# doing-science-to-stuff/ndt

Measured on AMD Instinct MI355X. Metric: Mray/s (primary+shadow+reflect) at 1920x1080, higher is better.
Workload: dtype f64

## Files before the change

ndt_amd/csrc/ndt_api.hip:

```cpp
#include "ndt_ctx.hpp"
#include <ctype.h>


static thread_local char g_err[512] = "";
int ndt_impl::fail(int code, const char *fmt, ...)
{
    va_list ap;
    va_start(ap, fmt);
    vsnprintf(g_err, sizeof(g_err), fmt, ap);
    va_end(ap);
    return code;
}

extern "C" const char *ndt_hip_last_error(void) { return g_err; }
extern "C" int ndt_hip_abi_version(void) { return NDT_HIP_ABI_VERSION; }

extern "C" int32_t ndt_hip_shard_rows(int32_t height, int32_t row_begin, int32_t row_step)
{
    if (row_step < 1 || row_begin < 0 || row_begin >= height) return 0;
    return (height - row_begin + row_step - 1) / row_step;
}

static const NdtKernelTable *table_for(int dims)
{
    switch (dims) {
    case 3: return ndt_kernel_table_3();
    case 4: return ndt_kernel_table_4();
    case 5: return ndt_kernel_table_5();
    case 6: return ndt_kernel_table_6();
    case 7: return ndt_kernel_table_7();
    case 8: return ndt_kernel_table_8();
    case 9: return ndt_kernel_table_9();
    case 10: return ndt_kernel_table_10();
    case 11: return ndt_kernel_table_11();
    case 12: return ndt_kernel_table_12();
    default: return nullptr;
    }
}

extern "C" int ndt_hip_create(int device, ndt_hip_ctx **out)
{
    if (!out) return fail(NDT_E_INVALID, "ndt_hip_create: out is NULL");
    *out = nullptr;
    int count = 0;
    hipError_t e = hipGetDeviceCount(&count);
    if (e != hipSuccess || count <= 0)
        return fail(NDT_E_DEVICE, "no HIP device available (%s); libndt_hip has no CPU path",
                    e == hipSuccess ? "device count is 0" : hipGetErrorString(e));
    if (device < 0 || device >= count) return fail(NDT_E_INVALID, "device %d out of range (have %d)", device, count);
    HIP_TRY(hipSetDevice(device));
    hipDeviceProp_t prop;
    HIP_TRY(hipGetDeviceProperties(&prop, device));
    if (strncmp(prop.gcnArchName, "gfx950", 6) != 0)
        return fail(NDT_E_DEVICE, "device %d is %s; this library carries gfx950 code objects only", device, prop.gcnArchName);
    ndt_hip_ctx *ctx = new ndt_hip_ctx();
    ctx->device = device;
    {
        static const char *const names[] = { "hybrid_level", "stream_below", "stream_below_list", "hull_box", "face_box", "face_tree", "face_groups", "item_sets", "gate_prepass", "gate_prepass_below", "item_boxes", "leaf_history", "leaf_scan", "leaf_scan_group", "multi_path", "sample_seed", "stream_fused", "fuse_primaries", "shade_pair", "light_overlap", "light_window", "debug_levels",
                                             "exit_probe", "shade_probe", "stream_probe", "test_small_pool" };
        const char *pl = getenv("NDT_HIP_PIPELINE");
        if (pl) (void)ndt_hip_set_option(ctx, "pipeline", !strcmp(pl, "levels") ? 1 : !strcmp(pl, "stream") ? 2 : !strcmp(pl, "hybrid") ? 3 : 0);
        for (const char *nm : names) {
            char env[64] = "NDT_HIP_";
            size_t k = strlen(env);
            for (const char *q = nm; *q && k + 1 < sizeof(env); ++q) env[k++] = (char)toupper((unsigned char)*q);
            env[k] = 0;
            const char *v = getenv(env);
            if (v && *v) (void)ndt_hip_set_option(ctx, nm, !strcmp(nm, "shade_probe") ? atoll(v) + 1 : atoll(v));
        }
        if (getenv("NDT_HIP_NO_HULL_BOX")) ctx->hull_box = false;
        if (getenv("NDT_HIP_NO_FACE_BOX")) ctx->face_box = false;
        if (getenv("NDT_HIP_NO_SHADE_PAIR") && atoi(getenv("NDT_HIP_NO_SHADE_PAIR"))) ctx->shade_pair = false;
    }
    e = hipStreamCreateWithFlags(&ctx->stream, hipStreamNonBlocking);
    if (e == hipSuccess) {
        int least = 0, greatest = 0;
        e = hipDeviceGetStreamPriorityRange(&least, &greatest);
        if (e == hipSuccess) e = hipStreamCreateWithPriority(&ctx->light_stream, hipStreamNonBlocking, least);
        if (e != hipSuccess) (void)hipStreamDestroy(ctx->stream);
    }
    if (e != hipSuccess) {
        delete ctx;
        return fail(NDT_E_DEVICE, "hipStreamCreate: %s", hipGetErrorString(e));
    }
    e = hipHostMalloc((void **)&ctx->h_counters, 128 * sizeof(int), hipHostMallocDefault);
    if (e == hipSuccess) e = hipHostMalloc((void **)&ctx->h_levels, (NDT_MAX_LEVELS + 1) * sizeof(LevelRange), hipHostMallocDefault);
    if (e == hipSuccess) e = hipHostMalloc((void **)&ctx->h_mail, (NDT_MAX_LEVELS + 2) * sizeof(LevelRange), hipHostMallocMapped | hipHostMallocCoherent);
    if (e == hipSuccess) e = hipHostMalloc((void **)&ctx->h_mail_tag, (NDT_MAX_LEVELS + 2) * sizeof(unsigned long long), hipHostMallocMapped | hipHostMallocCoherent);
    if (e == hipSuccess) e = hipHostGetDevicePointer((void **)&ctx->d_mail, ctx->h_mail, 0);
    if (e == hipSuccess) e = hipHostGetDevicePointer((void **)&ctx->d_mail_tag, ctx->h_mail_tag, 0);
    if (e == hipSuccess) memset(ctx->h_mail_tag, 0, (NDT_MAX_LEVELS + 2) * sizeof(unsigned long long));
    if (e == hipSuccess) e = hipHostMalloc((void **)&ctx->h_done, 16 * sizeof(unsigned long long), hipHostMallocMapped | hipHostMallocCoherent);
    if (e == hipSuccess) e = hipHostGetDevicePointer((void **)&ctx->d_done, ctx->h_done, 0);
    if (e == hipSuccess) memset(ctx->h_done, 0, 16 * sizeof(unsigned long long));
    if (e != hipSuccess) {
        (void)hipStreamDestroy(ctx->light_stream);
        (void)hipStreamDestroy(ctx->stream);
        delete ctx;
        return fail(NDT_E_DEVICE, "hipHostMalloc: %s", hipGetErrorString(e));
    }
    *out = ctx;
    return NDT_OK;
}

extern "C" int ndt_hip_destroy(ndt_hip_ctx *ctx)
{
    if (!ctx) return NDT_OK;
    worker_stop(ctx);
    (void)hipSetDevice(ctx->device);
    (void)sync_streams(ctx);
    free_workspace(ctx);
    free_stage(ctx);
    free_async(ctx);
    if (ctx->d_shard) (void)hipFree(ctx->d_shard);
    if (ctx->d_image) (void)hipFree(ctx->d_image);
    for (auto &slot : ctx->pool)
        if (slot.first) (void)hipFree(slot.first);
    for (auto &slot : ctx->pool2)
        if (slot.first) (void)hipFree(slot.first);
    if (ctx->d_blob) (void)hipFree(ctx->d_blob);
    if (ctx->d_out) (void)hipFree(ctx->d_out);
    if (ctx->d_fit) (void)hipFree(ctx->d_fit);
    free_kd(ctx);
    free_png(ctx);
    free_jpeg(ctx);
    free_depth(ctx);
    free_ssaa(ctx);
    if (ctx->d_eyes) (void)hipFree(ctx->d_eyes);
    if (ctx->h_counters) (void)hipHostFree(ctx->h_counters);
    if (ctx->h_levels) (void)hipHostFree(ctx->h_levels);
    if (ctx->h_mail) (void)hipHostFree(ctx->h_mail);
    if (ctx->h_mail_tag) (void)hipHostFree(ctx->h_mail_tag);
    if (ctx->h_done) (void)hipHostFree(ctx->h_done);
    for (hipEvent_t ev : ctx->ev_pool) (void)hipEventDestroy(ev);
    (void)hipStreamDestroy(ctx->light_stream);
    (void)hipStreamDestroy(ctx->stream);
    delete ctx;
    return NDT_OK;
}

extern "C" int ndt_hip_set_option(ndt_hip_ctx *ctx, const char *name, int64_t value)
{
    if (!ctx || !name) return fail(NDT_E_INVALID, "NULL argument");
    const bool on = value != 0;
    if (!strcmp(name, "pipeline")) {
        if (value < 0 || value > 3) return fail(NDT_E_INVALID, "pipeline %lld", (long long)value);
        ctx->pipeline = (int)value;
    } else if (!strcmp(name, "hybrid_level")) ctx->hybrid_level = (int)value;
    else if (!strcmp(name, "stream_below")) ctx->stream_below = value;
    else if (!strcmp(name, "stream_below_list")) ctx->stream_below_list = value;
    else if (!strcmp(name, "hull_box")) ctx->hull_box = on;
    else if (!strcmp(name, "face_box")) ctx->face_box = on;
    else if (!strcmp(name, "face_tree")) ctx->face_tree = on;
    else if (!strcmp(name, "face_groups")) ctx->face_groups = on;
    else if (!strcmp(name, "item_sets")) ctx->item_sets = on;
    else if (!strcmp(name, "item_boxes")) ctx->item_boxes = on;
    else if (!strcmp(name, "gate_prepass_below")) ctx->gate_prepass_below = value;
    else if (!strcmp(name, "gate_prepass")) ctx->gate_prepass = value < 0 ? 0 : value > 2 ? 2 : (int)value;
    else if (!strcmp(name, "sample_seed")) ctx->sample_seed = value;
    else if (!strcmp(name, "leaf_scan")) ctx->leaf_scan = on;
    else if (!strcmp(name, "leaf_scan_group")) ctx->leaf_scan_group = value < 1 ? 1 : value > 64 ? 64 : (int)value;
    else if (!strcmp(name, "leaf_history")) ctx->leaf_history = value < 0 ? 0 : value > 4 ? 4 : (int)value;
    else if (!strcmp(name, "multi_path")) {
        if (value < 0 || value > 2) return fail(NDT_E_INVALID, "multi_path %lld", (long long)value);
        ctx->multi_path = (int)value;
    } else if (!strcmp(name, "stream_fused")) ctx->stream_fused = on;
    else if (!strcmp(name, "fuse_primaries")) ctx->fuse_primaries = value < 0 ? -1 : on ? 1 : 0;
    else if (!strcmp(name, "shade_pair")) ctx->shade_pair = on;
    else if (!strcmp(name, "light_overlap")) ctx->light_overlap = on;
    else if (!strcmp(name, "light_window")) {
        if (value < 0 || value > 64) return fail(NDT_E_INVALID, "light_window %lld (0 auto, 1 .. 64)", (long long)value);
        ctx->light_window = (int)value;
        if (ctx->have_scene) light_windows(ctx);
    }
    else if (!strcmp(name, "debug_levels")) ctx->debug_levels = on;
    else if (!strcmp(name, "exit_probe")) ctx->exit_probe = on;
    else if (!strcmp(name, "shade_probe")) ctx->shade_probe = (int)value - 1;
    else if (!strcmp(name, "stream_probe")) ctx->stream_probe = on;
    else if (!strcmp(name, "test_small_pool")) ctx->test_small_pool = on;
    else return fail(NDT_E_INVALID, "unknown option '%s'", name);
    return NDT_OK;
}

extern "C" void *ndt_hip_stream(ndt_hip_ctx *ctx) { return ctx ? (void *)ctx->stream : nullptr; }
extern "C" int ndt_hip_synchronize(ndt_hip_ctx *ctx)
{
    if (!ctx) return fail(NDT_E_INVALID, "ctx is NULL");
    HIP_TRY(hipSetDevice(ctx->device));
    HIP_TRY(hipStreamSynchronize(ctx->stream));
    return NDT_OK;
}

extern "C" int ndt_hip_upload_scene(ndt_hip_ctx *ctx, const ndt_flat_scene *fs)
{
    if (!ctx || !fs) return fail(NDT_E_INVALID, "NULL argument");
    if (fs->abi_version != NDT_HIP_ABI_VERSION) return fail(NDT_E_INVALID, "scene ABI %d, library ABI %d", fs->abi_version, NDT_HIP_ABI_VERSION);
    if (fs->dims < NDT_MIN_DIMS || fs->dims > NDT_MAX_DIMS)
        return fail(NDT_E_UNSUPPORTED, "%d dimensions: kernels are built for %d..%d", fs->dims, NDT_MIN_DIMS, NDT_MAX_DIMS);
    if (fs->cam_type < 0 || fs->cam_type > 2) return fail(NDT_E_UNSUPPORTED, "camera type %d", fs->cam_type);
    if (fs->cam_type != 0 && (fs->cam_local_x_off < 0 || fs->cam_local_y_off < 0 || fs->cam_local_z_off < 0))
        return fail(NDT_E_INVALID, "VR / panorama cameras need the local axes (camera.h:69-71) in the flat scene");
    if (fs->n_lights < 0 || fs->n_lights > NDT_MAX_LIGHTS) return fail(NDT_E_UNSUPPORTED, "%d lights (max %d)", fs->n_lights, NDT_MAX_LIGHTS);
    if (fs->n_objects < 0 || fs->n_items < 0 || fs->n_items > fs->n_objects) return fail(NDT_E_INVALID, "object counts");
    if (fs->n_kd_nodes < 0 || fs->n_inf < 0 || fs->n_leaf_refs < 0) return fail(NDT_E_INVALID, "kd-tree counts");
    if (fs->n_objects > 0 && !fs->objects) return fail(NDT_E_INVALID, "objects is NULL");
    if (fs->n_lights > 0 && !fs->lights) return fail(NDT_E_INVALID, "lights is NULL");
    if (!fs->vecs) return fail(NDT_E_INVALID, "vecs is NULL");
    HIP_TRY(hipSetDevice(ctx->device));
    ctx->have_scene = false;
    int rc = build_blob(ctx, fs);
    if (rc) return rc;
    ctx->dims = fs->dims;
    ctx->kt = table_for(fs->dims);
    if (!ctx->kt) return fail(NDT_E_UNSUPPORTED, "no kernels for %d dimensions", fs->dims);
    HIP_TRY(sync_streams(ctx));
    if (ctx->d_blob_words < ctx->blob.size()) {
        if (ctx->d_blob) HIP_TRY(hipFree(ctx->d_blob));
        ctx->d_blob = nullptr;
        HIP_TRY(hipMalloc((void **)&ctx->d_blob, ctx->blob.size() * sizeof(double)));
        ctx->d_blob_words = ctx->blob.size();
    }
    HIP_TRY(hipMemcpyAsync(ctx->d_blob, ctx->blob.data(), ctx->blob.size() * sizeof(double), hipMemcpyHostToDevice, ctx->stream));
    HIP_TRY(hipStreamSynchronize(ctx->stream));
    ctx->aperture_radius = fs->cam_aperture_radius;
    ctx->have_scene = true;
    if (ctx->debug_levels)
        fprintf(stderr, "ndt_hip: scene blob: %d-D, %d items / %d objects, %d kd nodes of depth %d; %d words staged by the trace kernels (%d KB), %d in all; tier %d, %d mask word(s)\n",
                ctx->dims, ctx->sd.n_items, ctx->sd.n_objects, ctx->sd.n_kd_nodes, ctx->sd.kd_depth, ctx->sd.trace_words, ctx->sd.trace_words / 128,
                ctx->sd.total_words, ctx->tier, ctx->sd.mask_words);
    return NDT_OK;
}

__global__ void k_quantize(const double *rgba, unsigned char *out, long long n_values)
{
    const long long i = (long long)blockIdx.x * blockDim.x + threadIdx.x;
    if (i >= n_values) return;
    const double d = rgba[i];
    double m = (1.0 < d) ? 1.0 : d;
    m = (0.0 > m) ? 0.0 : m;
    out[i] = (unsigned char)(sqrt(m) * 255);
}

extern "C" int ndt_hip_quantize_device(ndt_hip_ctx *ctx, const void *d_rgba, void *d_rgba8, int64_t n_pixels)
{
    if (!ctx || !d_rgba || !d_rgba8 || n_pixels < 0) return fail(NDT_E_INVALID, "bad argument");
    HIP_TRY(hipSetDevice(ctx->device));
    const long long n = n_pixels * 4;
    if (n == 0) return NDT_OK;
    hipLaunchKernelGGL(k_quantize, dim3((unsigned)((n + 255) / 256)), dim3(256), 0, ctx->stream, (const double *)d_rgba,
                       (unsigned char *)d_rgba8, n);
    HIP_TRY(hipGetLastError());
    return NDT_OK;
// ... 77 lines not shown
```

ndt_amd/csrc/ndt_ctx.hpp:

```cpp
#pragma once
#include <hip/hip_runtime.h>
#include <hip/hip_ext.h>
#include <math.h>
#include <stdarg.h>
#include <stdio.h>
#include <stdlib.h>
#include <string.h>
#include <time.h>
#include <functional>
#include <string>
#include <vector>

#include "../../include/ndt_hip.h"
#include "ndt_kernels.hpp"

namespace ndt_impl {

struct CtxWorker;

int fail(int code, const char *fmt, ...) __attribute__((format(printf, 2, 3)));

}
using namespace ndt_impl;

// ... 8 lines not shown
    size_t bounds_bytes = 0, refs_bytes = 0, nodes_bytes = 0, slices_bytes = 0, slice_off_bytes[2] = { 0, 0 }, totals_bytes = 0;
    std::vector<ndt_flat_kdnode> nodes;
    std::vector<int32_t> leaf_refs, inf_refs;
    std::vector<double> bb_lower, bb_upper;
    int dims = 0, depth = 0, launches = 0, grows = 0;
    bool valid = false;
};

struct PngState {
    void *d_rgba8 = nullptr, *d_filtered = nullptr, *d_row_filter = nullptr, *d_slots = nullptr, *d_meta = nullptr, *d_offsets = nullptr,
         *d_file = nullptr, *d_info = nullptr;
    size_t rgba8_bytes = 0, filtered_bytes = 0, row_filter_bytes = 0, slots_bytes = 0, meta_bytes = 0, offsets_bytes = 0, file_bytes = 0,
           info_bytes = 0;
    void *h_info = nullptr;
};

struct JpegState {
    void *d_rgba8 = nullptr, *d_coef = nullptr, *d_slots = nullptr, *d_meta = nullptr, *d_offsets = nullptr, *d_file = nullptr, *d_info = nullptr;
    size_t rgba8_bytes = 0, coef_bytes = 0, slots_bytes = 0, meta_bytes = 0, offsets_bytes = 0, file_bytes = 0, info_bytes = 0;
    void *h_info = nullptr;
};

struct DepthState {
    void *d_records = nullptr;
    void *d_rgba8 = nullptr, *d_depth8 = nullptr;
    size_t records_bytes = 0, rgba8_bytes = 0, depth8_bytes = 0;
    void *h_result = nullptr;
    int launches = 0;
    double finish_ms = 0.0;
};

struct SsaaState {
    void *d_pass = nullptr;
    void *d_acc = nullptr;
    void *d_rgba8 = nullptr, *d_depth8 = nullptr;
    size_t pass_bytes = 0, acc_bytes = 0, rgba8_bytes = 0, depth8_bytes = 0;
    hipEvent_t ev[16] = {};
    int launches = 0;
    int factor = 0;
    double fold_ms = 0.0;
};

struct ndt_hip_ctx {
    int device = 0;
    hipStream_t stream = nullptr;
    hipStream_t light_stream = nullptr;
    const NdtKernelTable *kt = nullptr;
    int dims = 0;
    bool have_scene = false;
    double aperture_radius = 0.0;
    int cam_type = 0;
    bool have_eyes = false, have_local_axes = false;
    bool has_area_lights = false;
    SceneDesc sd{};
    std::vector<double> blob;
    double *d_blob = nullptr;
    size_t d_blob_words = 0;
    int tier = 0;
    int n_shadow_lights = 0;
    struct LightWindow {
        int first, count;
        int n_seg;
        unsigned long long ambient_bits;
    };
    int light_window = 0;
    std::vector<int> light_types;
    std::vector<LightWindow> windows;
    Workspace ws{};
    std::vector<void *> ws_allocs;
    std::vector<void *> sa_allocs;
    std::vector<std::pair<void *, size_t>> pool;
    std::vector<std::pair<void *, size_t>> pool2;
    long long ws_dims = 0;
    long long ws_slab_words = 0;
    int ws_nseg = 0;
    int pipeline = 0;
    int hybrid_level = 2;
    long long stream_below = 1000000;
    long long stream_below_list = 30000;
    StreamArgs sa{};
    bool stream_probe = false, exit_probe = false, debug_levels = false, test_small_pool = false;
    bool hull_box = true, face_box = true, shade_pair = true;
    bool light_overlap = true;
    bool face_tree = true;
    bool face_groups = true;
    int fuse_primaries = -1;
    bool stream_fused = true;
    bool item_sets = true;
    int gate_prepass = 2;
    long long gate_prepass_below = 400000;
    bool item_boxes = true;
    int leaf_scan_group = 64;
    bool leaf_scan = true;
    int leaf_history = 4;
    int shade_probe = -1;
    long long sa_cap = 0, sa_sh_cap = 0;
    int sa_nseg = 0;
    void *d_eyes = nullptr;
    size_t d_eyes_bytes = 0;
    void *d_fit = nullptr;
    size_t d_fit_bytes = 0;
    int fit_launches = 0;
    KdState kd;
    PngState png;
    JpegState jpeg;
    DepthState depth;
    SsaaState ssaa;
    void *d_out = nullptr;
    size_t d_out_bytes = 0;
    void *d_shard = nullptr;
    size_t d_shard_bytes = 0;
    void *d_image = nullptr;
    size_t d_image_bytes = 0;
    void *d_rgba8[2] = { nullptr, nullptr };
    size_t d_rgba8_bytes[2] = { 0, 0 };
    hipStream_t copy_stream = nullptr;
    hipEvent_t ev_quantised[2] = { nullptr, nullptr }, ev_copied[2] = { nullptr, nullptr };
    bool copy_pending[2] = { false, false };
    int rgba8_turn = 0;
    void *d_stage = nullptr;
    size_t d_stage_bytes = 0;
    hipStream_t stage_stream = nullptr;
    int stage_device = 0;
    long long sample_seed = 0;
    int multi_path = 0;
    int multi_path_taken = 0;
    ndt_impl::CtxWorker *worker = nullptr;
    int *h_counters = nullptr;
    LevelRange *h_levels = nullptr;
    LevelRange *h_mail = nullptr;
    unsigned long long *h_mail_tag = nullptr;
    LevelRange *d_mail = nullptr;
    unsigned long long *d_mail_tag = nullptr;
    unsigned long long frame_tag = 0;
    unsigned long long *h_done = nullptr;
    unsigned long long *d_done = nullptr;
    std::vector<hipEvent_t> ev_pool;
};

namespace ndt_impl {

struct HullFaces {
    std::vector<double> rows;
    std::vector<unsigned long long> possible;
    int n_faces = 0;
};
bool hcube_hull_box(const ndt_flat_scene *fs, const ndt_flat_object &o, int n, std::vector<double> &rows, HullFaces *faces = nullptr);
void hcube_face_tree(const HullFaces &hf, int n, std::vector<double> &rows, std::vector<int> &level_off, int &top);
void hcube_face_groups(const HullFaces &hf, const std::vector<double> &hull_rows, int n, std::vector<double> &clusters, std::vector<int> &table,
                       std::vector<int> &face_set, std::vector<int> &members);
bool scene_item_boxes(const ndt_flat_scene *fs, int n, std::vector<double> &frame, std::vector<double> &rows, std::vector<char> &has);
int build_blob(ndt_hip_ctx *ctx, const ndt_flat_scene *fs);
void light_windows(ndt_hip_ctx *ctx);
SceneDesc window_desc(const ndt_hip_ctx *ctx, const SceneDesc &sd, int k);

void free_workspace(ndt_hip_ctx *ctx);
hipError_t sync_streams(ndt_hip_ctx *ctx);
int ensure_workspace(ndt_hip_ctx *ctx, long long cap, long long sh_cap);
int render_pass(ndt_hip_ctx *ctx, RenderGeom rg, bool prof, void *d_rgba, ndt_render_stats &st, void *d_depth = nullptr);
void launch_fill_black(hipStream_t s, double *rgba, long long n_pixels);
void add_stats(ndt_render_stats &acc, const ndt_render_stats &st);

void print_stream_probe(const unsigned int *wave_log, float kernel_ms);
void print_shade_probe(const unsigned int *shade_log, int shade_probe, long long finish_waves);
void print_exit_probe(const unsigned int *exit_log, int launches);
void print_phase_timing(const unsigned long long *dbg);
// ... 109 lines not shown
```

ndt_amd/csrc/ndt_finish.hpp:

```cpp
#pragma once
#include "ndt_kernels.hpp"

template <bool COH> __device__ __forceinline__ double fin_ld(const double *p)
{
    if (COH)
        return __longlong_as_double((long long)__hip_atomic_load(reinterpret_cast<unsigned long long *>(const_cast<double *>(p)),
                                                                 __ATOMIC_RELAXED, __HIP_MEMORY_SCOPE_AGENT));
    return *p;
}
template <bool COH> __device__ __forceinline__ int fin_ldi(const int *p)
{
    if (COH) return __hip_atomic_load(const_cast<int *>(p), __ATOMIC_RELAXED, __HIP_MEMORY_SCOPE_AGENT);
    return *p;
}

template <bool COH>
__device__ __forceinline__ unsigned long long finish_pixel(const double *blob, const SceneDesc &sd, const Workspace &ws, const RenderGeom &rg,
                                                           int N_, long long g, double *rgba, double *depth_out)
{
    long long out_idx = g;
    if (!rg.samples) {
        const int tile = (int)(g >> 6), lane = (int)(g & 63);
        const int px = (tile % rg.tiles_x) * 8 + (lane & 7);
        const int py = (tile / rg.tiles_x) * 8 + (lane >> 3);
        out_idx = (long long)py * rg.width + px;
    }
    const double l[4] = { fin_ld<COH>(ws.clr + 0 * ws.cap + g), fin_ld<COH>(ws.clr + 1 * ws.cap + g), fin_ld<COH>(ws.clr + 2 * ws.cap + g),
                          fin_ldi<COH>(ws.hit_obj + g) >= 0 ? 1.0 : blob[sd.off_cam + 4 * N_ + 7] };
    double t[4] = { 0.0, 0.0, 0.0, 0.0 };
    const double max_diff = 1.0 / 256.0;
    double clr_diff = 256;
    int samples = 0;
    const double gb0 = (fabs(l[1]) > fabs(l[2])) ? fabs(l[1]) : fabs(l[2]);
    const double lmax = (fabs(l[0]) > gb0) ? fabs(l[0]) : gb0;
    const bool finite = lmax <= 1.0e300;
    for (int i = 0; i < 1 || (!rg.raw_samples && i < 10000 && clr_diff > max_diff); ++i) {
        if (i > 1) {
            const double ii = (double)i * (double)(i - 1);
            const double est = lmax / ii;
            const double band = 1.0e-15 * (8.0 * (double)i * (double)i) + 1.0e-12;
            if (finite && est > max_diff * (1.0 + band)) {
                clr_diff = est;
            } else if (finite && est < max_diff * (1.0 - band)) {
                clr_diff = est;
            } else {
                const double dr = fabs(t[0] / (i - 1) - (t[0] + l[0]) / i);
                const double dg = fabs(t[1] / (i - 1) - (t[1] + l[1]) / i);
                const double db = fabs(t[2] / (i - 1) - (t[2] + l[2]) / i);
                const double gb = (dg > db) ? dg : db;
                clr_diff = (dr > gb) ? dr : gb;
            }
        }
        t[0] += l[0]; t[1] += l[1]; t[2] += l[2]; t[3] += l[3];
        samples += 1;
    }
    double *out = rgba + out_idx * 4;
    out[0] = t[0] / samples;
    out[1] = t[1] / samples;
    out[2] = t[2] / samples;
    out[3] = t[3] / samples;
    if (depth_out) depth_out[out_idx] = fin_ld<COH>(ws.depth + g);
    return (unsigned long long)samples * (unsigned long long)fin_ldi<COH>(ws.count + g);
}
```

ndt_amd/csrc/ndt_frame.hip:

```cpp
#include "ndt_ctx.hpp"
#include "ndt_finish.hpp"
#include <stddef.h>

static void free_stream_args(ndt_hip_ctx *ctx)
{
    for (void *p : ctx->sa_allocs) (void)hipFree(p);
    ctx->sa_allocs.clear();
    memset(&ctx->sa, 0, sizeof(ctx->sa));
    ctx->sa_cap = ctx->sa_sh_cap = 0;
    ctx->sa_nseg = 0;
}

hipError_t ndt_impl::sync_streams(ndt_hip_ctx *ctx)
{
    const hipError_t e = hipStreamSynchronize(ctx->stream);
    if (e != hipSuccess || !ctx->light_stream) return e;
    return hipStreamSynchronize(ctx->light_stream);
}

void ndt_impl::free_workspace(ndt_hip_ctx *ctx)
{
    for (void *p : ctx->ws_allocs) (void)hipFree(p);
    ctx->ws_allocs.clear();
    free_stream_args(ctx);
// ... 170 lines not shown
            }
        ctl[k] = v;
    }
    for (long long k = i; k < node_batches; k += stride) {
        sa.node_fill[k] = 0;
        sa.sh_pending[k] = 0;
        for (int sh = 0; sh < NDT_PRIM_SHARDS; ++sh) sa.sec_ring[(long long)sh * node_batches + k] = 0;
        sa.fin_ring[k] = 0;
    }
    for (long long k = i; k < sh_batches; k += stride) {
        sa.sh_fill[k] = 0;
        sa.sh_ring[k] = 0;
    }
    if (frame_too) {
        for (long long k = i; k < 64 * 8; k += stride) ws.ref_rays[k] = 0ull;
        for (long long k = i; k < 4; k += stride) ws.counters[k] = 0;
    }
}

__global__ void k_stream_done(Workspace ws, StreamArgs sa, unsigned long long *done, unsigned long long tag)
{
    const int lane = threadIdx.x;
    unsigned long long ref = ws.ref_rays[8 * lane];
    for (int d = 32; d > 0; d >>= 1) ref += __shfl_xor(ref, d, 64);
    if (lane != 0) return;
    const StreamCtl *c = sa.ctl;
    done[0] = (unsigned long long)(long long)c->node_tail.v;
    done[1] = (unsigned long long)(long long)c->overflow.v;
    done[2] = (unsigned long long)(long long)(c->abort.v | (c->timeout_where.v << 8));
    done[3] = (unsigned long long)(long long)c->n_shadow.v;
    done[4] = (unsigned long long)(long long)(c->max_level.v + 1);
    done[5] = ref;
    done[6] = (unsigned long long)(long long)c->n_children.v;
    __threadfence_system();
    __hip_atomic_store(&done[7], tag, __ATOMIC_RELEASE, __HIP_MEMORY_SCOPE_SYSTEM);
}

__device__ __forceinline__ void resolve_node(const double *blob, const SceneDesc &sd, const Workspace &ws, int specular, long long g)
{
    if (ws.depth_left[g] <= 0) return;
    const int obj = ws.hit_obj[g];
    if (obj < 0) return;
    const int mw = sd.off_mat + 8 * obj;
    const double hitr[3] = { blob[mw + 3], blob[mw + 4], blob[mw + 5] };
    double c[3] = { ws.clr[0 * ws.cap + g], ws.clr[1 * ws.cap + g], ws.clr[2 * ws.cap + g] };
    int cnt = ws.count[g];
    const int refl = ws.child_refl[g];
    if (refl != -1) {
        double ref[3] = { 0.0, 0.0, 0.0 };
        if (refl >= 0) {
            ref[0] = ws.clr[0 * ws.cap + refl]; ref[1] = ws.clr[1 * ws.cap + refl]; ref[2] = ws.clr[2 * ws.cap + refl];
            cnt += ws.count[refl];
        }
        for (int k = 0; k < 3; ++k) {
            if (specular) c[k] = (1 - hitr[k]) * (c[k]) + (hitr[k]) * ref[k];
            else c[k] += hitr[k] * ref[k];
        }
    }
    const int refr = ws.child_refr[g];
    if (refr != -1) {
        double ref[3] = { 0.0, 0.0, 0.0 };
        if (refr >= 0) {
            ref[0] = ws.clr[0 * ws.cap + refr]; ref[1] = ws.clr[1 * ws.cap + refr]; ref[2] = ws.clr[2 * ws.cap + refr];
            cnt += ws.count[refr];
        }
        for (int k = 0; k < 3; ++k) c[k] += (1.0 - hitr[k]) * ref[k];
    }
    ws.clr[0 * ws.cap + g] = c[0];
    ws.clr[1 * ws.cap + g] = c[1];
    ws.clr[2 * ws.cap + g] = c[2];
    ws.count[g] = cnt;
}

__global__ void __launch_bounds__(256) k_resolve(const double *blob, SceneDesc sd, Workspace ws, int specular, int level)
{
    const LevelRange lr = ws.levels[level];
    for (long long r = (long long)blockIdx.x * blockDim.x + threadIdx.x; r < lr.count; r += (long long)gridDim.x * blockDim.x)
        resolve_node(blob, sd, ws, specular, lr.begin + r);
}

#ifndef NDT_FINISH_BLOCK
#define NDT_FINISH_BLOCK 256
#endif
__global__ void __launch_bounds__(NDT_FINISH_BLOCK) k_finish_pixels(const double *blob, SceneDesc sd, Workspace ws, RenderGeom rg, int N_,
                                                       double *rgba, double *depth_out, int resolve0)
{
    const long long g = (long long)blockIdx.x * blockDim.x + threadIdx.x;
    unsigned long long weighted = 0ull;
    if (resolve0 && g < rg.n_primary) resolve_node(blob, sd, ws, rg.specular, g);
    if (g < rg.n_primary && ws.depth_left[g] > 0) weighted = finish_pixel<false>(blob, sd, ws, rg, N_, g, rgba, depth_out);
    for (int d = 32; d > 0; d >>= 1) weighted += __shfl_down(weighted, d, 64);
    if ((threadIdx.x & 63) == 0 && weighted) atomicAdd(ws.ref_rays + 8 * ((blockIdx.x * (NDT_FINISH_BLOCK / 64) + (threadIdx.x >> 6)) & 63), weighted);
}

__global__ void k_fill_black(double *rgba, long long n_pixels)
{
    const long long i = (long long)blockIdx.x * blockDim.x + threadIdx.x;
    if (i >= n_pixels) return;
    rgba[4 * i + 0] = 0.0; rgba[4 * i + 1] = 0.0; rgba[4 * i + 2] = 0.0; rgba[4 * i + 3] = 1.0;
}

void ndt_impl::launch_fill_black(hipStream_t s, double *rgba, long long n_pixels)
{
    hipLaunchKernelGGL(k_fill_black, dim3((unsigned)((n_pixels + 255) / 256)), dim3(256), 0, s, rgba, n_pixels);
}

void ndt_impl::add_stats(ndt_render_stats &acc, const ndt_render_stats &st)
{
    acc.rays_primary += st.rays_primary;
    acc.rays_secondary += st.rays_secondary;
    acc.rays_shadow += st.rays_shadow;
    acc.rays_ref_equiv += st.rays_ref_equiv;
    if (st.levels > acc.levels) acc.levels = st.levels;
    acc.trace_launches += st.trace_launches;
    acc.trace_ms += st.trace_ms;
    acc.frame_ms += st.frame_ms;
    if (st.node_capacity > acc.node_capacity) acc.node_capacity = st.node_capacity;
}


static hipEvent_t get_event(ndt_hip_ctx *ctx, size_t idx)
{
    while (ctx->ev_pool.size() <= idx) {
        hipEvent_t ev;
        if (hipEventCreate(&ev) != hipSuccess) return nullptr;
        ctx->ev_pool.push_back(ev);
    }
    return ctx->ev_pool[idx];
}

static double wall_s()
{
    struct timespec ts;
    clock_gettime(CLOCK_MONOTONIC, &ts);
    return (double)ts.tv_sec + 1e-9 * (double)ts.tv_nsec;
}

static int wait_for_tag(ndt_hip_ctx *ctx, const unsigned long long *word, unsigned long long tag, const char *what, int bounce = 0)
{
    const double t_wait = wall_s();
    while (__atomic_load_n(word, __ATOMIC_ACQUIRE) != tag) {
        if (wall_s() - t_wait > 30.0) {
            HIP_TRY(hipStreamSynchronize(ctx->stream));
            if (__atomic_load_n(word, __ATOMIC_ACQUIRE) != tag) return fail(NDT_E_STATE, what, bounce);
        }
    }
    return NDT_OK;
}

static long long n_pixels(const RenderGeom &rg) { return rg.samples ? (long long)rg.n_samples : (long long)rg.rows * rg.width; }

template <typename Kernel, typename... Args>
static void launch_stamped(Kernel k, dim3 grid, dim3 block, hipStream_t s, hipEvent_t ev_start, hipEvent_t ev_stop, Args... args)
{
    if (ev_start || ev_stop)
        hipExtLaunchKernelGGL(k, grid, block, 0, s, ev_start, ev_stop, 0u, args...);
    else
        hipLaunchKernelGGL(k, grid, block, 0, s, args...);
}

static void launch_finish_pixels(ndt_hip_ctx *ctx, const SceneDesc &sd_pass, const Workspace &ws, const RenderGeom &rg, void *d_rgba, void *d_depth,
                                 int resolve0)
{
    hipLaunchKernelGGL(k_finish_pixels, dim3((unsigned)((rg.n_primary + NDT_FINISH_BLOCK - 1) / NDT_FINISH_BLOCK)), dim3(NDT_FINISH_BLOCK), 0, ctx->stream,
                       ctx->d_blob, sd_pass, ws, rg, ctx->dims, (double *)d_rgba, (double *)d_depth, resolve0);
}

static int stream_roots(ndt_hip_ctx *ctx, bool prof, long long begin, long long count, int primaries, StreamArgs &sa)
{
    sa = ctx->sa;
    sa.root_begin = (int)(begin & ~63LL);
    sa.n_primary = (int)(((begin + count + 63) & ~63LL) - sa.root_begin);
    sa.valid_begin = (int)begin;
    sa.valid_end = (int)(begin + count);
    sa.roots_are_primaries = primaries;
    sa.fused = 0;
    if (!prof) sa.wave_log = nullptr;
    else if (sa.wave_log) HIP_TRY(hipMemsetAsync(sa.wave_log, 0, (size_t)24 * NDT_STREAM_LOG_WAVES * sizeof(unsigned int), ctx->stream));
    return NDT_OK;
}

static void launch_stream_init(ndt_hip_ctx *ctx, const Workspace &ws, const StreamArgs &sa, int frame_too, hipEvent_t ev_start)
{
    const long long sh_batches = (long long)sa.n_seg * (sa.seg_cap / 64) + NDT_STREAM_LOG_WAVES;
    launch_stamped(k_stream_init, dim3(512), dim3(256), ctx->stream, ev_start, nullptr, ws, sa, (long long)sa.node_batches, sh_batches, frame_too);
}

static const int PASS_AGAIN = 1;

static int render_pass_stream(ndt_hip_ctx *ctx, const RenderGeom &rg, const SceneDesc &sd_pass, bool prof, void *d_rgba, void *d_depth, long long cap,
                              long long sh_cap, ndt_render_stats &st, bool &no_room)
{
    hipStream_t s = ctx->stream;
    const NdtKernelTable *kt = ctx->kt;
    const int n_seg = ctx->n_shadow_lights > 0 ? ctx->n_shadow_lights : 1;
    for (int attempt = 0; attempt < 8; ++attempt) {
        if (sh_cap < cap * n_seg) sh_cap = cap * n_seg;
        int rc = NDT_OK;
        if (cap > 0x7fffff00LL || sh_cap > 0x7fffff00LL) rc = fail(NDT_E_NOMEM, "ray tree exceeds 2^31 nodes");
        if (!rc) rc = ensure_workspace(ctx, cap, sh_cap);
        if (!rc) rc = ensure_stream_args(ctx);
        no_room = rc == NDT_E_NOMEM;
        if (rc) return rc;
        const Workspace ws = ctx->ws;
        StreamArgs sa;
        if ((rc = stream_roots(ctx, prof, 0, rg.n_primary, 1, sa))) return rc;
        sa.fused = ctx->stream_fused ? 1 : 0;
        sa.rgba = (double *)d_rgba;
        sa.depth_out = (double *)d_depth;
        hipEvent_t ev_begin = nullptr, ev_end = nullptr, ev_k0 = nullptr, ev_k1 = nullptr;
        if (prof) {
            ev_begin = get_event(ctx, 0);
            ev_end = get_event(ctx, 1);
            ev_k0 = get_event(ctx, 2);
            ev_k1 = get_event(ctx, 3);
        }
        const unsigned long long tag = ++ctx->frame_tag;
        launch_stream_init(ctx, ws, sa, 1, ev_begin);
        if (!sa.fused) kt->primary(s, ctx->d_blob, sd_pass, ws, rg);
        kt->frame_stream(s, ctx->d_blob, sd_pass, ws, rg, sa, ctx->tier, ctx->sd.mask_words, ev_k0, ev_k1);
        if (!sa.fused) launch_finish_pixels(ctx, sd_pass, ws, rg, d_rgba, d_depth, 0);
        launch_stamped(k_stream_done, dim3(1), dim3(64), s, nullptr, ev_end, ws, sa, ctx->d_done, tag);
        HIP_TRY(hipGetLastError());
        if ((rc = wait_for_tag(ctx, &ctx->h_done[7], tag, "the frame never completed"))) return rc;
        if (prof) HIP_TRY(hipEventSynchronize(ev_end));
        const int overflow = (int)(long long)ctx->h_done[1], aborted = (int)(long long)ctx->h_done[2];
        if (overflow != 0) {
            if (overflow & 1) cap *= 2;
            if (overflow & 2) sh_cap *= 2;
            continue;
        }
        if (aborted != 0)
            return fail(NDT_E_STATE, "the frame kernel gave up (abort %d, where %d): a work item never arrived", aborted & 0xff, aborted >> 8);
        st = ndt_render_stats{};
        st.rays_primary = n_pixels(rg);
        st.rays_secondary = (long long)ctx->h_done[6];
        st.rays_shadow = (long long)ctx->h_done[3];
        st.rays_ref_equiv = (long long)ctx->h_done[5];
        st.levels = (int)ctx->h_done[4];
        st.trace_launches = 1;
        st.node_capacity = ws.cap;
        if (prof) {
            float km = 0, fm = 0;
            HIP_TRY(hipEventElapsedTime(&km, ev_k0, ev_k1));
            HIP_TRY(hipEventElapsedTime(&fm, ev_begin, ev_end));
            st.trace_ms = km;
            st.frame_ms = fm;
            if (sa.wave_log) print_stream_probe(sa.wave_log, km);
        }
        return NDT_OK;
    }
    return fail(NDT_E_NOMEM, "ray-tree workspace kept overflowing");
}

struct FrameInFlight {
    ndt_hip_ctx *ctx;
    const RenderGeom &rg;
    const SceneDesc &sd_pass;
    const bool prof;
    const bool hybrid;
    void *d_rgba, *d_depth;
    hipStream_t s;
    const NdtKernelTable *kt;
    Workspace ws;
    const int n_levels;
    const int hand;
    const int n_win;
    const bool windowed;
    const bool overlap;
    hipStream_t ls;
    hipEvent_t ev_lit[3] = { nullptr, nullptr, nullptr };
    int light_next = 0;
    hipEvent_t light_tail = nullptr;
    std::vector<SceneDesc> sd_win;
    int win_emits = 0;
    unsigned long long tag = 0;
    int slots = 0, queue_slot = 0;
    int launches = 0;
    size_t ev_n = 0;
    hipEvent_t ev_begin = nullptr, ev_end = nullptr, ev_k0 = nullptr, ev_k1 = nullptr;
    std::vector<std::pair<hipEvent_t, hipEvent_t>> trace_ev;
    std::vector<std::string> trace_dbg;
    int shade_launch = 0;
    long long shade_probe_finish_waves = 0;
    int n_run;
    std::vector<long long> level_nodes;
    int pending_finish = -1;
    long long pending_upper = 0;
    bool resolve_with_finish = false;
    StreamArgs sa{};
    bool streamed = false;

    FrameInFlight(ndt_hip_ctx *c, const RenderGeom &g, const SceneDesc &sd, bool p, bool hyb, void *rgba, void *depth)
        : ctx(c), rg(g), sd_pass(sd), prof(p), hybrid(hyb), d_rgba(rgba), d_depth(depth), s(c->stream), kt(c->kt), ws(c->ws),
          n_levels(g.max_depth > 1 ? g.max_depth : 1), hand(hyb ? c->hybrid_level : n_levels + 1), n_win((int)c->windows.size()),
          windowed(n_win > 1), overlap(c->light_overlap && !windowed && !hyb), ls(c->light_stream), n_run(n_levels)
    {
        ws.mail = ctx->d_mail;
        ws.mail_tag = ctx->d_mail_tag;
        for (int k = 0; windowed && k < n_win; ++k) sd_win.push_back(window_desc(ctx, sd_pass, k));
    }

    int render(long long &cap, long long &sh_cap, ndt_render_stats &st);
    int render_frame(long long &cap, long long &sh_cap, ndt_render_stats &st);
    int frame_init(long long &sh_cap);
    int traced(TraceJob &tj, const std::string &what, const SceneDesc *sd_job = nullptr);
    int answer_bank(int b) const { return overlap ? b % 3 : 0; }
    Workspace shade_ws(long long finish_nodes, int b, hipStream_t on);
    int trace_primaries();
    void light_and_shade(int b, long long upper);
    int light_beside(int b);
    hipError_t join_light();
    int trace_bounce(int b, long long upper);
    int trace_windows(int b, long long upper);
    void light_last();
    int hand_off(long long &cap);
    void resolve();
    int close();
    int report(long long &cap, long long &sh_cap, ndt_render_stats &st);
    hipError_t print_debug(int levels_used);
};

int FrameInFlight::render(long long &cap, long long &sh_cap, ndt_render_stats &st)
{
    const int rc = render_frame(cap, sh_cap, st);
    const hipError_t e = join_light();
    if (rc == NDT_OK && e != hipSuccess) return fail(NDT_E_DEVICE, "joining the light stream: %s", hipGetErrorString(e));
    return rc;
}

hipError_t FrameInFlight::join_light()
{
    if (!light_tail) return hipSuccess;
    const hipError_t e = hipStreamWaitEvent(s, light_tail, 0);
    light_tail = nullptr;
    return e;
}

int FrameInFlight::light_beside(int b)
{
    kt->shade_finish(ls, ctx->d_blob, sd_pass, shade_ws(level_nodes[b], b, ls), rg, b, level_nodes[b], 0);
    HIP_TRY(hipEventRecord(ev_lit[b % 3], ls));
    light_tail = ev_lit[b % 3];
    light_next = b + 1;
    return NDT_OK;
}

int FrameInFlight::render_frame(long long &cap, long long &sh_cap, ndt_render_stats &st)
{
    int rc;
    if ((rc = frame_init(sh_cap))) return rc;
    if ((rc = trace_primaries())) return rc;
    long long upper = rg.n_primary;
    for (int b = 0; b < n_levels && b < hand; ++b) {
        if ((windowed ? b + 2 : queue_slot + 1) > NDT_QUEUE_SLOTS || b + 1 > NDT_MAX_LEVELS)
            return fail(NDT_E_UNSUPPORTED, "more than %d bounces", NDT_QUEUE_SLOTS - 1);
        if (b > 0) {
            if ((rc = wait_for_tag(ctx, &ctx->h_mail_tag[b], tag, "bounce %d was never published", b))) return rc;
            upper = ctx->h_mail[b].count;
            if (overlap && b >= 2 && (rc = light_beside(b - 2))) return rc;
            if (upper <= 0) {
                n_run = b;
                break;
            }
        }
        level_nodes.push_back(upper);
        light_and_shade(b, upper);
        if ((rc = trace_bounce(b, upper))) return rc;
        if (windowed && (rc = trace_windows(b, upper))) return rc;
        pending_finish = b;
        pending_upper = upper;
    }
    light_last();
    if (overlap && n_run >= 2 && light_next == n_run - 2) {
        if ((rc = wait_for_tag(ctx, &ctx->h_mail_tag[n_run], tag, "bounce %d was never published", n_run))) return rc;
        if ((rc = light_beside(n_run - 2))) return rc;
    }
    if (hybrid && n_run >= hand && hand < n_levels && (rc = hand_off(cap))) return rc;
    HIP_TRY(join_light());
    resolve();
    launch_finish_pixels(ctx, sd_pass, ws, rg, d_rgba, d_depth, n_run >= 1 ? 1 : 0);
    if ((rc = close())) return rc;
    return report(cap, sh_cap, st);
}

int FrameInFlight::frame_init(long long &sh_cap)
{
    if (prof) {
        ev_begin = get_event(ctx, ev_n++);
        ev_end = get_event(ctx, ev_n++);
    }
    for (int p = 0; overlap && p < 3; ++p)
        if (!(ev_lit[p] = get_event(ctx, ev_n++))) return fail(NDT_E_DEVICE, "hipEventCreate failed");
    if (prof && ctx->exit_probe)
        HIP_TRY(hipMemsetAsync(ws.exit_log, 0, (size_t)NDT_EXIT_LOG_LAUNCHES * NDT_EXIT_LOG_WORDS * sizeof(unsigned int), s));
    tag = ++ctx->frame_tag;
    LevelRange level0;
    level0.begin = 0;
    level0.count = rg.n_primary;
    level0.seg_stride = (rg.n_primary + 63) & ~63LL;
    level0.n_shadow = 0;
    if ((long long)ctx->n_shadow_lights * level0.seg_stride > ws.sh_cap) {
        sh_cap = (long long)ctx->n_shadow_lights * level0.seg_stride;
        return PASS_AGAIN;
    }
    const long long want_slots = (long long)n_levels * (windowed ? n_win : 1) + 2;
    slots = want_slots > NDT_QUEUE_SLOTS ? NDT_QUEUE_SLOTS : (int)want_slots;
    launch_stamped(k_frame_init, dim3(8), dim3(256), s, ev_begin, nullptr, ws, rg.n_primary, level0, slots * NDT_QUEUE_INTS);
    if (windowed) HIP_TRY(hipMemsetAsync(ws.counters + NDT_CNT_WIN, 0, (NDT_CNT_ALLOC - NDT_CNT_WIN) * sizeof(int), s));
    return NDT_OK;
}

int FrameInFlight::traced(TraceJob &tj, const std::string &what, const SceneDesc *sd_job)
{
    tj.queue = ws.counters + NDT_CNT_QUEUE + (queue_slot % NDT_QUEUE_SLOTS) * NDT_QUEUE_INTS;
    if (queue_slot++ >= slots) HIP_TRY(hipMemsetAsync(tj.queue, 0, NDT_QUEUE_INTS * sizeof(int), s));
    const SceneDesc &sdj = sd_job ? *sd_job : sd_pass;
    tj.exit_log = (ctx->exit_probe && prof && launches < NDT_EXIT_LOG_LAUNCHES) ? ws.exit_log + (size_t)launches * NDT_EXIT_LOG_WORDS : nullptr;
    hipEvent_t a = nullptr, b2 = nullptr;
    if (prof) {
        a = get_event(ctx, ev_n++);
        b2 = get_event(ctx, ev_n++);
        trace_ev.push_back({ a, b2 });
        trace_dbg.push_back(what);
    }
    kt->trace(s, ctx->d_blob, sdj, ws, tj, ctx->tier, ctx->sd.mask_words, a, b2);
    ++launches;
    return NDT_OK;
}

Workspace FrameInFlight::shade_ws(long long finish_nodes, int b, hipStream_t on)
{
    Workspace w = ws;
    w.sobj += answer_bank(b) * ws.sh_cap;
    w.sprim += answer_bank(b) * ws.sh_cap;
    if (shade_launch++ != ctx->shade_probe || !prof) {
        w.shade_log = nullptr;
    } else {
        shade_probe_finish_waves = (finish_nodes + 255) / 256 * 4;
        (void)hipMemsetAsync(w.shade_log, 0, (size_t)2 * NDT_SHADE_LOG_WAVES * sizeof(unsigned int), on);
    }
    return w;
}

static void job_closest(TraceJob &tj, const Workspace &ws)
{
    tj.dense.o = ws.ray_o; tj.dense.v = ws.ray_v; tj.dense.stride = ws.cap; tj.dense.lim = nullptr;
    tj.dense.valid = ws.depth_left; tj.dense.out_obj = ws.hit_obj; tj.dense.out_prim = ws.hit_prim;
    tj.begin = 0;
}

static void job_shadow(TraceJob &tj, const Workspace &ws, const SceneDesc &sd_pass, int b, long long upper, int n_seg, const int *seg_count,
                       int bank = 0)
{
    tj.n_seg = n_seg;
    tj.seg.o = ws.so; tj.seg.v = ws.sv; tj.seg.stride = ws.sh_cap; tj.seg.lim = ws.slim; tj.seg.valid = nullptr;
    tj.seg_light_origins = sd_pass.light_origins;
    tj.seg.out_obj = ws.sobj + bank * ws.sh_cap; tj.seg.out_prim = ws.sprim + bank * ws.sh_cap;
    tj.seg_count = seg_count;
    tj.seg_stride = (upper + 63) & ~63LL;
    tj.levels = ws.levels;
    tj.seg_level = b;
}

int FrameInFlight::trace_primaries()
{
    const bool fuse_primaries = (ctx->fuse_primaries < 0 ? ctx->dims >= 4 : ctx->fuse_primaries != 0) && ctx->cam_type == 0;
    if (!fuse_primaries) kt->primary(s, ctx->d_blob, sd_pass, ws, rg);
    TraceJob tj{};
    job_closest(tj, ws);
    tj.count = rg.n_primary;
    tj.publish_level = -1;
    if (fuse_primaries) {
        tj.make_primaries = 1;
        tj.rg = rg;
    }
// ... 223 lines not shown
```

Before: 4347.

## Finish missed primary pixels early on the light stream during bounce tracing

```diff
diff --git a/ndt_amd/csrc/ndt_api.hip b/ndt_amd/csrc/ndt_api.hip
--- a/ndt_amd/csrc/ndt_api.hip
+++ b/ndt_amd/csrc/ndt_api.hip
@@ -56,7 +56,7 @@
     ndt_hip_ctx *ctx = new ndt_hip_ctx();
     ctx->device = device;
     {
-        static const char *const names[] = { "hybrid_level", "stream_below", "stream_below_list", "hull_box", "face_box", "face_tree", "face_groups", "item_sets", "gate_prepass", "gate_prepass_below", "item_boxes", "leaf_history", "leaf_scan", "leaf_scan_group", "multi_path", "sample_seed", "stream_fused", "fuse_primaries", "shade_pair", "light_overlap", "light_window", "debug_levels",
+        static const char *const names[] = { "hybrid_level", "stream_below", "stream_below_list", "hull_box", "face_box", "face_tree", "face_groups", "item_sets", "gate_prepass", "gate_prepass_below", "item_boxes", "leaf_history", "leaf_scan", "leaf_scan_group", "multi_path", "sample_seed", "stream_fused", "fuse_primaries", "shade_pair", "light_overlap", "early_pixels", "light_window", "debug_levels",
                                              "exit_probe", "shade_probe", "stream_probe", "test_small_pool" };
         const char *pl = getenv("NDT_HIP_PIPELINE");
         if (pl) (void)ndt_hip_set_option(ctx, "pipeline", !strcmp(pl, "levels") ? 1 : !strcmp(pl, "stream") ? 2 : !strcmp(pl, "hybrid") ? 3 : 0);
@@ -168,6 +168,10 @@
     else if (!strcmp(name, "fuse_primaries")) ctx->fuse_primaries = value < 0 ? -1 : on ? 1 : 0;
     else if (!strcmp(name, "shade_pair")) ctx->shade_pair = on;
     else if (!strcmp(name, "light_overlap")) ctx->light_overlap = on;
+    else if (!strcmp(name, "early_pixels")) {
+        if (value < 0 || value > 2) return fail(NDT_E_INVALID, "early_pixels %lld (0 off, 1 missed primaries, 2 and childless ones)", (long long)value);
+        ctx->early_pixels = (int)value;
+    }
     else if (!strcmp(name, "light_window")) {
         if (value < 0 || value > 64) return fail(NDT_E_INVALID, "light_window %lld (0 auto, 1 .. 64)", (long long)value);
         ctx->light_window = (int)value;
diff --git a/ndt_amd/csrc/ndt_ctx.hpp b/ndt_amd/csrc/ndt_ctx.hpp
--- a/ndt_amd/csrc/ndt_ctx.hpp
+++ b/ndt_amd/csrc/ndt_ctx.hpp
@@ -114,6 +114,7 @@
     bool stream_probe = false, exit_probe = false, debug_levels = false, test_small_pool = false;
     bool hull_box = true, face_box = true, shade_pair = true;
     bool light_overlap = true;
+    int early_pixels = 1;
     bool face_tree = true;
     bool face_groups = true;
     int fuse_primaries = -1;
diff --git a/ndt_amd/csrc/ndt_finish.hpp b/ndt_amd/csrc/ndt_finish.hpp
--- a/ndt_amd/csrc/ndt_finish.hpp
+++ b/ndt_amd/csrc/ndt_finish.hpp
@@ -12,6 +12,16 @@
 {
     if (COH) return __hip_atomic_load(const_cast<int *>(p), __ATOMIC_RELAXED, __HIP_MEMORY_SCOPE_AGENT);
     return *p;
+}
+
+#define NDT_PART_REST 0
+#define NDT_PART_MISSED 1
+#define NDT_PART_CHILDLESS 2
+__device__ __forceinline__ int pixel_part(const Workspace &ws, long long g)
+{
+    if (ws.depth_left[g] <= 0) return NDT_PART_REST;
+    if (ws.hit_obj[g] < 0) return NDT_PART_MISSED;
+    return (ws.child_refl[g] == -1 && ws.child_refr[g] == -1) ? NDT_PART_CHILDLESS : NDT_PART_REST;
 }
 
 template <bool COH>
diff --git a/ndt_amd/csrc/ndt_frame.hip b/ndt_amd/csrc/ndt_frame.hip
--- a/ndt_amd/csrc/ndt_frame.hip
+++ b/ndt_amd/csrc/ndt_frame.hip
@@ -276,6 +276,12 @@
 #ifndef NDT_FINISH_BLOCK
 #define NDT_FINISH_BLOCK 256
 #endif
+__device__ __forceinline__ void add_ref_rays(const Workspace &ws, unsigned long long weighted)
+{
+    for (int d = 32; d > 0; d >>= 1) weighted += __shfl_down(weighted, d, 64);
+    if ((threadIdx.x & 63) == 0 && weighted) atomicAdd(ws.ref_rays + 8 * ((blockIdx.x * (NDT_FINISH_BLOCK / 64) + (threadIdx.x >> 6)) & 63), weighted);
+}
+
 __global__ void __launch_bounds__(NDT_FINISH_BLOCK) k_finish_pixels(const double *blob, SceneDesc sd, Workspace ws, RenderGeom rg, int N_,
                                                        double *rgba, double *depth_out, int resolve0)
 {
@@ -283,8 +289,19 @@
     unsigned long long weighted = 0ull;
     if (resolve0 && g < rg.n_primary) resolve_node(blob, sd, ws, rg.specular, g);
     if (g < rg.n_primary && ws.depth_left[g] > 0) weighted = finish_pixel<false>(blob, sd, ws, rg, N_, g, rgba, depth_out);
-    for (int d = 32; d > 0; d >>= 1) weighted += __shfl_down(weighted, d, 64);
-    if ((threadIdx.x & 63) == 0 && weighted) atomicAdd(ws.ref_rays + 8 * ((blockIdx.x * (NDT_FINISH_BLOCK / 64) + (threadIdx.x >> 6)) & 63), weighted);
+    add_ref_rays(ws, weighted);
+}
+
+__global__ void __launch_bounds__(NDT_FINISH_BLOCK) k_finish_part(const double *blob, SceneDesc sd, Workspace ws, RenderGeom rg, int N_,
+                                                     double *rgba, double *depth_out, int resolve0, int take)
+{
+    const long long g = (long long)blockIdx.x * blockDim.x + threadIdx.x;
+    unsigned long long weighted = 0ull;
+    if (g < rg.n_primary && ((take >> pixel_part(ws, g)) & 1)) {
+        if (resolve0) resolve_node(blob, sd, ws, rg.specular, g);
+        if (ws.depth_left[g] > 0) weighted = finish_pixel<false>(blob, sd, ws, rg, N_, g, rgba, depth_out);
+    }
+    add_ref_rays(ws, weighted);
 }
 
 __global__ void k_fill_black(double *rgba, long long n_pixels)
@@ -358,6 +375,13 @@
 {
     hipLaunchKernelGGL(k_finish_pixels, dim3((unsigned)((rg.n_primary + NDT_FINISH_BLOCK - 1) / NDT_FINISH_BLOCK)), dim3(NDT_FINISH_BLOCK), 0, ctx->stream,
                        ctx->d_blob, sd_pass, ws, rg, ctx->dims, (double *)d_rgba, (double *)d_depth, resolve0);
+}
+
+static void launch_finish_part(ndt_hip_ctx *ctx, hipStream_t on, const SceneDesc &sd_pass, const Workspace &ws, const RenderGeom &rg, void *d_rgba,
+                               void *d_depth, int resolve0, int take)
+{
+    hipLaunchKernelGGL(k_finish_part, dim3((unsigned)((rg.n_primary + NDT_FINISH_BLOCK - 1) / NDT_FINISH_BLOCK)), dim3(NDT_FINISH_BLOCK), 0, on,
+                       ctx->d_blob, sd_pass, ws, rg, ctx->dims, (double *)d_rgba, (double *)d_depth, resolve0, take);
 }
 
 static int stream_roots(ndt_hip_ctx *ctx, bool prof, long long begin, long long count, int primaries, StreamArgs &sa)
@@ -466,6 +490,9 @@
     hipEvent_t ev_lit[3] = { nullptr, nullptr, nullptr };
     int light_next = 0;
     hipEvent_t light_tail = nullptr;
+    const int early;
+    int early_done = 0;
+    hipEvent_t ev_early = nullptr;
     std::vector<SceneDesc> sd_win;
     int win_emits = 0;
     unsigned long long tag = 0;
@@ -488,7 +515,8 @@
     FrameInFlight(ndt_hip_ctx *c, const RenderGeom &g, const SceneDesc &sd, bool p, bool hyb, void *rgba, void *depth)
         : ctx(c), rg(g), sd_pass(sd), prof(p), hybrid(hyb), d_rgba(rgba), d_depth(depth), s(c->stream), kt(c->kt), ws(c->ws),
           n_levels(g.max_depth > 1 ? g.max_depth : 1), hand(hyb ? c->hybrid_level : n_levels + 1), n_win((int)c->windows.size()),
-          windowed(n_win > 1), overlap(c->light_overlap && !windowed && !hyb), ls(c->light_stream), n_run(n_levels)
+          windowed(n_win > 1), overlap(c->light_overlap && !windowed && !hyb), ls(c->light_stream), early(overlap ? c->early_pixels : 0),
+          n_run(n_levels)
     {
         ws.mail = ctx->d_mail;
         ws.mail_tag = ctx->d_mail_tag;
@@ -504,6 +532,8 @@
     int trace_primaries();
     void light_and_shade(int b, long long upper);
     int light_beside(int b);
+    int early_pixels_beside(int part);
+    int mark_light_tail(hipEvent_t ev);
     hipError_t join_light();
     int trace_bounce(int b, long long upper);
     int trace_windows(int b, long long upper);
@@ -534,9 +564,28 @@
 int FrameInFlight::light_beside(int b)
 {
     kt->shade_finish(ls, ctx->d_blob, sd_pass, shade_ws(level_nodes[b], b, ls), rg, b, level_nodes[b], 0);
-    HIP_TRY(hipEventRecord(ev_lit[b % 3], ls));
-    light_tail = ev_lit[b % 3];
+    int rc;
+    if (b == 0 && early >= 2 && (rc = early_pixels_beside(NDT_PART_CHILDLESS))) return rc;
+    if ((rc = mark_light_tail(ev_lit[b % 3]))) return rc;
     light_next = b + 1;
+    return NDT_OK;
+}
+
+int FrameInFlight::early_pixels_beside(int part)
+{
+    launch_finish_part(ctx, ls, sd_pass, ws, rg, d_rgba, d_depth, 0, 1 << part);
+    early_done |= 1 << part;
+    return part == NDT_PART_MISSED ? mark_light_tail(ev_early) : NDT_OK;
+}
+
+int FrameInFlight::mark_light_tail(hipEvent_t ev)
+{
+    const hipError_t e = hipEventRecord(ev, ls);
+    if (e != hipSuccess) {
+        (void)hipStreamSynchronize(ls);
+        return fail(NDT_E_DEVICE, "hipEventRecord on the light stream: %s", hipGetErrorString(e));
+    }
+    light_tail = ev;
     return NDT_OK;
 }
 
@@ -552,6 +601,7 @@
         if (b > 0) {
             if ((rc = wait_for_tag(ctx, &ctx->h_mail_tag[b], tag, "bounce %d was never published", b))) return rc;
             upper = ctx->h_mail[b].count;
+            if (early >= 1 && b == 1 && (rc = early_pixels_beside(NDT_PART_MISSED))) return rc;
             if (overlap && b >= 2 && (rc = light_beside(b - 2))) return rc;
             if (upper <= 0) {
                 n_run = b;
@@ -573,7 +623,8 @@
     if (hybrid && n_run >= hand && hand < n_levels && (rc = hand_off(cap))) return rc;
     HIP_TRY(join_light());
     resolve();
-    launch_finish_pixels(ctx, sd_pass, ws, rg, d_rgba, d_depth, n_run >= 1 ? 1 : 0);
+    if (early_done) launch_finish_part(ctx, s, sd_pass, ws, rg, d_rgba, d_depth, n_run >= 1 ? 1 : 0, 7 & ~early_done);
+    else launch_finish_pixels(ctx, sd_pass, ws, rg, d_rgba, d_depth, n_run >= 1 ? 1 : 0);
     if ((rc = close())) return rc;
     return report(cap, sh_cap, st);
 }
@@ -586,6 +637,7 @@
     }
     for (int p = 0; overlap && p < 3; ++p)
         if (!(ev_lit[p] = get_event(ctx, ev_n++))) return fail(NDT_E_DEVICE, "hipEventCreate failed");
+    if (early && !(ev_early = get_event(ctx, ev_n++))) return fail(NDT_E_DEVICE, "hipEventCreate failed");
     if (prof && ctx->exit_probe)
         HIP_TRY(hipMemsetAsync(ws.exit_log, 0, (size_t)NDT_EXIT_LOG_LAUNCHES * NDT_EXIT_LOG_WORDS * sizeof(unsigned int), s));
     tag = ++ctx->frame_tag;
```

Measured after the change: 4420, median of 6. 1.7% higher.
